# bd4/gpu-mpi-tests

Measured on AMD Instinct MI355X. Metric: 2D 5-pt Jacobi stencil MLUPS (fp64), higher is better.
Workload: dtype fp64; 1 GPU; model=mpi_stencil2d jacobi5 32768x32768 fp64, global_batch=1073741824, parallelism=spatial2d py1 x px1, serial, engine=native, hipgraph=False, temporal_blocking=True, sweeps_per_pass=20, pass_plan=98x20+1x1, exact_levels=False, init=random, transport=none, halo_bytes_per_rank=0, device=cuda:0

## Files before the change

csrc/kernels/jacobi5tb.hpp:

```cpp
#pragma once
#include <hip/hip_runtime.h>

#include <algorithm>
#include <cstdio>
#include <cstdlib>
#include <atomic>
#include <map>
#include <mutex>
#include <string>
#include <utility>
#include <vector>

#include "common.hpp"
#include "gmt/kernels.h"
#include "gmt/tb_geom.h"

namespace gmt {
namespace tb {

constexpr int kMaxRect = 8;
constexpr int kMaxThreads = 512;
constexpr uint32_t kDrop = 0x80000000u;

constexpr int unroll_for(int NL) { return NL > 1 ? 2 * (NL - 1) + 1 : 2; }
// ... 52 lines not shown
  using C = Cfg<K>;
  return static_cast<int64_t>(C::HS) * Sh<K, NW>::ROWG + static_cast<int64_t>(NW) * C::RS * C::ROW;
}

struct Args {
  int64_t r[kMaxRect][4];
  int64_t nstrip[kMaxRect];
  int64_t tstart[kMaxRect + 1];
  int64_t dom[4];
  int64_t ld;
  int64_t last_row;
  int n;
  int mask;
  int64_t e0[kMaxRect], e1[kMaxRect], nmid[kMaxRect], lmid[kMaxRect];
  int64_t nmid_b[kMaxRect], lmid_b[kMaxRect];
  int nw;
  double quarter;
  int64_t sig_wgs;
  unsigned* sig_count;
  uint64_t* signal;
  int prio;
  int rb_rect;
  int rb_s, rb_n;
  int64_t sig_rows, sig_total, sig_dispatch;
  int64_t edges_last;
  int sh;
  int shmap;
  int col_keep;
  int cb_rect;
  int cb_lo, cb_hi;
// ... 144 lines not shown
    else if constexpr (J == 2) GMT_KC("v_mov_b64 %[v2], %[c]");
    else GMT_KC("v_mov_b64 %[v3], %[c]");
  } else {
    if constexpr (J == 0) GMT_KC("v_mul_f64 %[v0], %[c], 4.0");
    else if constexpr (J == 1) GMT_KC("v_mul_f64 %[v1], %[c], 4.0");
    else if constexpr (J == 2) GMT_KC("v_mul_f64 %[v2], %[c], 4.0");
    else GMT_KC("v_mul_f64 %[v3], %[c], 4.0");
  }
#undef GMT_KC
}

#ifndef GMT_TB_SKIP_DEAD
#define GMT_TB_SKIP_DEAD 1
#endif

template <int K, int J, bool EXACT, bool EDGE, int RULE, bool UP, int PUSH, int SH>
__device__ __forceinline__ void run_stage(const Args& a, const double* __restrict__ u, double* __restrict__ un,
                                          char* ring, int lane, int64_t xs, int64_t xe, int64_t ys, int64_t ye,
                                          int nsteps, int sig_step, int xd, int64_t cf, int hdelta, uint64_t hm0,
                                          uint64_t hm1) {
  using C = Cfg<K>;
  constexpr int NC = C::NC;
  constexpr int PB = J * C::NL + 1, PE = (J + 1) * C::NL;
  constexpr bool kIn = J == 0;
  constexpr bool kOut = J == C::S - 1;
  constexpr bool SYNC = C::S > 1;
  constexpr int kP = C::P, kRS = C::RS, kHS = C::HS;
  constexpr uint32_t kRow = C::ROW;
  constexpr int D = C::DLAG * J;
  constexpr int kGroups = 1 + (PUSH & 1) + ((PUSH >> 1) & 1) + (PUSH == 3 ? 1 : 0);
  constexpr int SPS = kOut ? (EDGE ? NC : kGroups * (NC / 2)) : 0;
  static_assert(!(PUSH && EDGE), "inline halo exchange: no odd-edge stores");
  constexpr bool kDma = kIn;
  constexpr int DPS = kDma ? C::NDMA : 0;
  char* const hand_rd = ring + kRS * kRow + (J > 0 ? J - 1 : 0) * kHS * kRow;
// ... 123 lines not shown
  static_assert(RULE < 2 || kColSlot < NC, "column slot");
  const int64_t gcol = !gw && cf <= dx0 - 1 && dx0 - 1 < cf + C::COLS ? dx0 - 1 : dx1;
  const uint64_t kcm = RULE >= 2 ? __builtin_amdgcn_ballot_w64(c0 + kColSlot == gcol) : 0;

  const int64_t yanchor = up ? ye - 1 + K : yl;
  const auto clamp32 = [](int64_t x) {
    return static_cast<int>(x < INT32_MIN ? int64_t{INT32_MIN} : x > INT32_MAX ? int64_t{INT32_MAX} : x);
  };
  int tlo = up ? (gn ? INT32_MIN : clamp32(yanchor - dy1 + 1)) : (gs ? INT32_MIN : clamp32(dy0 - yanchor));
  int thi = up ? (gs ? INT32_MAX : clamp32(yanchor - dy0 + 1)) : (gn ? INT32_MAX : clamp32(dy1 - yanchor));
  if constexpr (PUSH != 0 && SH != 0) {
    tlo = __builtin_amdgcn_readfirstlane(tlo);
    thi = __builtin_amdgcn_readfirstlane(thi);
  }
  const uint32_t span = static_cast<uint32_t>(thi) - static_cast<uint32_t>(tlo);
  auto level = [&](const dv<NC>& up_, const dv<NC>& c, const dv<NC>& dn, int t) -> dv<NC> {
#pragma clang fp contract(off)
    const double w = dpp_from_lower(c.c[NC - 1]), e = dpp_from_upper(c.c[0]);
    dv<NC> v;
    static_for<0, NC>([&](auto Q) {
#pragma clang fp contract(off)
      constexpr int j = decltype(Q)::value;
      double l, r;
      if constexpr (j == 0) l = w;
      else l = c.c[j - 1];
      if constexpr (j == NC - 1) r = e;
      else r = c.c[j + 1];
      if constexpr (EXACT) v.c[j] = quarter * ((l + r) + (up_.c[j] + dn.c[j]));
      else v.c[j] = (l + r) + (up_.c[j] + dn.c[j]);
    });
    if constexpr (RULE >= 2) {
      keep_col<EXACT, kColSlot, NC>(v, c.c[kColSlot], kcm);
    } else if constexpr (RULE == 1) {
      keep_cells<EXACT, NC>(v, c, kxm, static_cast<uint32_t>(t) - static_cast<uint32_t>(tlo), span);
    }
    return v;
  };

  constexpr int NL = PE - PB + 1;
  dv<NC> W[NL > 1 ? NL - 1 : 1][2];
#pragma unroll
  for (int p = 0; p < (NL > 1 ? NL - 1 : 1); ++p)
#pragma unroll
    for (int j = 0; j < 2; ++j) W[p][j] = dv_zero<NC>();

  if constexpr (kIn) {
    static_for<0, kP>([&](auto I) {
      store_step(decltype(I)::value - kP, dv_zero<NC>());
// ... 10 lines not shown
      r2 = lds_row<NC>(ring + (s % kRS) * kRow, lane);
    } else {
      if constexpr (SH) {
        r0 = lds_row_sh<NC, kQS>(hsh + ((s + kHS - 4) % kHS) * kRowG);
        r1 = lds_row_sh<NC, kQS>(hsh + ((s + kHS - 3) % kHS) * kRowG);
        r2 = lds_row_sh<NC, kQS>(hsh + ((s + kHS - 2) % kHS) * kRowG);
      } else {
        r0 = lds_row<NC>(hand_rd + ((s + kHS - 4) % kHS) * kRow, lane);
        r1 = lds_row<NC>(hand_rd + ((s + kHS - 3) % kHS) * kRow, lane);
        r2 = lds_row<NC>(hand_rd + ((s + kHS - 2) % kHS) * kRow, lane);
      }
    }
  };
  load_rows(0);

  auto step = [&](auto Jc, int s) {
    constexpr int j = decltype(Jc)::value;
    (void)j;
    dv<NC> v = level(r0, r1, r2, s - D - PB);
    __builtin_amdgcn_sched_barrier(0);
    static_for<PB + 1, PE + 1>([&](auto Q) {
      constexpr int p = decltype(Q)::value;
      const dv<NC> nv = level(W[p - 1 - PB][0], W[p - 1 - PB][1], v, s - D - p);
      W[p - 1 - PB][0] = W[p - 1 - PB][1];
      W[p - 1 - PB][1] = v;
      v = nv;
      __builtin_amdgcn_sched_barrier(0);
    });
    if constexpr (kOut) {
      if constexpr (!EXACT) {
#pragma unroll
        for (int q = 0; q < NC; ++q) v.c[q] = __builtin_amdgcn_ldexp(v.c[q], -2 * K);
      }
      store_step(s, v);
    } else if constexpr (SH) {
      lds_put_sh<NC, kQS>(hsh + (s % kHS) * kRowG, v, hm0, hm1);
    } else {
      lds_put<NC>(hand_wr + (s % kHS) * kRow, lane, v);
// ... 2 lines not shown
    if constexpr (SYNC) asm volatile("s_waitcnt lgkmcnt(0)" ::: "memory");
    load_rows(s + 1);
    if constexpr (SYNC) asm volatile("s_barrier" ::: "memory");
  };

  constexpr int kU = C::U;
  constexpr bool kSkip0 = GMT_TB_SKIP_DEAD && !kIn && SYNC && kU <= D + 2 * PB;
  int s_first = 0;
  if constexpr (kSkip0) {
    for (int s = 0; s < kU - 1; ++s) step_barrier();
    asm volatile("s_waitcnt lgkmcnt(0)" ::: "memory");
    load_rows(kU);
    asm volatile("s_barrier" ::: "memory");
    s_first = kU;
  }
  for (int s0 = s_first; s0 < nsteps; s0 += kU) {
    static_for<0, kU>([&](auto Jc) { step(Jc, s0 + decltype(Jc)::value); });
    if constexpr (kOut) {
      if (static_cast<unsigned>(sig_step - s0) < static_cast<unsigned>(kU)) {
        asm volatile("s_waitcnt vmcnt(0)" ::: "memory");
        __builtin_amdgcn_fence(__ATOMIC_RELEASE, "agent");
        if (lane == 0 && __hip_atomic_fetch_add(a.sig_count, 1u, __ATOMIC_ACQ_REL, __HIP_MEMORY_SCOPE_AGENT) ==
                             static_cast<unsigned>(a.sig_total - 1)) {
          __hip_atomic_store(a.sig_count, 0u, __ATOMIC_RELAXED, __HIP_MEMORY_SCOPE_AGENT);
          __hip_atomic_fetch_add(a.signal, uint64_t{1}, __ATOMIC_RELEASE, __HIP_MEMORY_SCOPE_AGENT);
        }
      }
    }
  }
  wait_vmcnt<0>();
}

template <int K, bool EXACT, bool EDGE, bool PUSH, int SH>
__device__ __forceinline__ void tb_block(const Args& a, const double* __restrict__ u, double* __restrict__ un,
                                         int64_t t) {
  using C = Cfg<K>;
  constexpr int G = C::S;
  extern __shared__ d2 lds_dyn[];
  const int lane = threadIdx.x & (kWave - 1);
  const int wave = __builtin_amdgcn_readfirstlane(static_cast<int>(threadIdx.x) / kWave);
  const bool smaj = G > 1 && a.shmap;
  const int sl = smaj ? wave % a.nw : wave / G, stage = smaj ? wave / a.nw : wave % G;
  int k = 0;
  while (k + 1 < a.n && t >= a.tstart[k + 1]) ++k;
  const int64_t lt = t - a.tstart[k];
  const int64_t ngroups = (a.nstrip[k] + a.nw - 1) / a.nw;
  const int64_t ry0 = a.r[k][2], ry1 = a.r[k][2] + a.r[k][3];
  const int64_t e0 = a.e0[k], e1 = a.e1[k];
  const int64_t nedge = (e0 > 0) + (e1 > 0);
  const int rbs = k == a.rb_rect ? a.rb_s : 0, rbn = k == a.rb_rect ? a.rb_n : 0, rb = rbs + rbn;
  const int cblo = k == a.cb_rect ? a.cb_lo : 0;
  const int cbhi = k == a.cb_rect && ngroups > 1 ? a.cb_hi : 0;
  const int64_t ncb = (cblo || (k == a.cb_rect && a.cb_hi && ngroups == 1)) + cbhi;
  const int64_t nsb = nedge + a.nmid_b[k];
  const int64_t ng = ngroups - ncb;
  const int64_t cbf = ncb > 0 && (cblo || ngroups == 1) ? 1 : 0;
  const bool b0 = cbf == 0, b1 = ngroups > 1 && !cbhi;
  const int64_t nbnd = (b0 ? 1 : 0) + (b1 ? 1 : 0);
  const int64_t n_cb = ncb * nsb, n_rb = rb * ng, n_ed = nedge * ng, n_bd = (a.nmid_b[k] - rb) * nbnd;
  int64_t gi, m = -1;
  int edge = 0, dir = 1;
  bool band = false;
  auto seg_of = [&](int64_t sg, int64_t nm) {
    if (e0 > 0 && sg == 0) {
      edge = 0;
    } else if (sg < (e0 > 0) + nm) {
      m = sg - (e0 > 0);
    } else {
      edge = 1;
    }
  };
  if (lt < n_cb) {
    const int64_t c = lt / nsb;
    gi = (c == 0 && cbf) ? 0 : ngroups - 1;
    seg_of(lt % nsb, a.nmid_b[k]);
  } else if (lt < n_cb + n_rb) {
    const int64_t l0 = lt - n_cb;
    gi = cbf + l0 % ng;
    const bool north = l0 >= ng || !rbs;
    const int64_t nm = (gi == 0 || gi == ngroups - 1) ? a.nmid_b[k] : a.nmid[k];
    m = north ? nm - 1 : 0;
    dir = north ? -1 : 1;
    band = true;
  } else if (lt < n_cb + n_rb + n_ed) {
    const int64_t l1 = lt - n_cb - n_rb;
    edge = (l1 / ng == 0 && e0 > 0) ? 0 : 1;
    gi = cbf + l1 % ng;
  } else if (lt < n_cb + n_rb + n_ed + n_bd) {
    const int64_t l2 = lt - n_cb - n_rb - n_ed;
    m = rbs + l2 / nbnd;
    gi = (l2 % nbnd == 0 && b0) ? 0 : ngroups - 1;
  } else {
    const int64_t l3 = lt - n_cb - n_rb - n_ed - n_bd;
    m = rbs + l3 / (ngroups - 2);
    gi = 1 + l3 % (ngroups - 2);
  }
  const int64_t nm = (gi == 0 || gi == ngroups - 1) ? a.nmid_b[k] : a.nmid[k];
  int64_t ys, ye;
  if (m < 0) {
    ys = edge == 0 ? ry0 : ry1 - e1;
    ye = edge == 0 ? ry0 + e0 : ry1;
  } else {
    const int64_t mid = ry1 - e1 - (ry0 + e0);
    ys = ry0 + e0 + m * mid / nm;
    ye = ry0 + e0 + (m + 1) * mid / nm;
  }
  constexpr int kU = C::U;
  const int sig_step = band ? static_cast<int>(C::LAG + 2 * K + a.sig_rows - 1) : -1;
  const int nsteps = static_cast<int>((ye - ys + 2 * K + C::LAG + kU - 1) / kU * kU);
  const int64_t strip = gi * a.nw + sl;
  if (strip >= a.nstrip[k]) {
    if constexpr (G > 1) {
      for (int s = 0; s < nsteps; ++s) step_barrier();
    }
    return;
  }
  constexpr int64_t wout = C::WOUT;
  const int64_t rx0 = a.r[k][0], rx1 = a.r[k][0] + a.r[k][1];
  int64_t xs, xe, cf;
  char* ring;
// ... 18 lines not shown
    } else {
      off = H::O + H::S1 * sl;
      xs = gx + H::S1 * sl;
      xe = sl < H::NW - 1 ? xs + H::S1 : gx + H::GOUT;
    }
    cf = ga + off;
    hdelta = static_cast<int>(4 * off - (ring - lds));
  } else {
    xs = rx0 + strip * wout;
    if (xs + wout > rx1) xs = rx1 - wout > rx0 ? rx1 - wout : rx0;
    xe = xs + wout < rx1 ? xs + wout : rx1;
    cf = xs - C::KL;
    ring = reinterpret_cast<char*>(lds_dyn) + sl * strip_lds<K>();
  }
  const int64_t cx0 = cf, cx1 = cx0 + C::COLS;
  const bool rule = (cx0 < a.dom[0] && !(a.mask & 1)) || (cx1 > a.dom[0] + a.dom[1] && !(a.mask & 2)) ||
                    (ys - K < a.dom[2] && !(a.mask & 4)) || (ye + K > a.dom[2] + a.dom[3] && !(a.mask & 8));
  int rule_kind = rule ? 1 : 0;
  constexpr bool kColBodies = SH && !PUSH;
  constexpr int kJW = SH ? Sh<K, SH ? SH : 4>::kJW : 3, kJE = SH ? Sh<K, SH ? SH : 4>::kJE : 0;
  if constexpr (kColBodies) {
    const bool ry = (ys - K < a.dom[2] && !(a.mask & 4)) || (ye + K > a.dom[2] + a.dom[3] && !(a.mask & 8));
    const int64_t gw0 = a.dom[0] - 1, ge0 = a.dom[0] + a.dom[1];
    const bool hw = !(a.mask & 1) && cx0 <= gw0 && gw0 < cx1, he = !(a.mask & 2) && cx0 <= ge0 && ge0 < cx1;
    if (rule && !ry && hw != he && a.col_keep) {
      const int jslot = static_cast<int>(((hw ? gw0 : ge0) - cx0) & 3);
      if (jslot == kJW || jslot == kJE) rule_kind = 2 + jslot;
    }
  }
  const bool pw = PUSH && (a.push[GMT_PUSH_W] || a.push[GMT_PUSH_SW] || a.push[GMT_PUSH_NW]);
  const bool pe = PUSH && (a.push[GMT_PUSH_E] || a.push[GMT_PUSH_SE] || a.push[GMT_PUSH_NE]);
  const int xd = !PUSH ? -1 : (strip == 0 && pw) ? GMT_PUSH_W : (strip == a.nstrip[k] - 1 && pe) ? GMT_PUSH_E : -1;
  const bool py = PUSH && (((a.push[GMT_PUSH_S] || a.push[GMT_PUSH_SW] || a.push[GMT_PUSH_SE]) &&
                            ys < a.dom[2] + a.push_w) ||
                           ((a.push[GMT_PUSH_N] || a.push[GMT_PUSH_NW] || a.push[GMT_PUSH_NE]) &&
                            ye > a.dom[2] + a.dom[3] - a.push_w));
  const int pm = (xd >= 0 ? 1 : 0) | (py ? 2 : 0);
  using T = std::true_type;
  using F = std::false_type;
  auto go = [&](auto jc, auto rule_c, auto up_c, int sstep) __attribute__((always_inline)) {
    constexpr int j = decltype(jc)::value;
    auto run = [&](auto push_c) __attribute__((always_inline)) {
      run_stage<K, j, EXACT, EDGE, decltype(rule_c)::value, decltype(up_c)::value, decltype(push_c)::value, SH>(
          a, u, un, ring, lane, xs, xe, ys, ye, nsteps, sstep, xd, cf, hdelta, hm0, hm1);
    };
    using P0 = std::integral_constant<int, 0>;
    if constexpr (PUSH && j == G - 1) {
      if (pm != 0) run(std::integral_constant<int, 3>{});
      else run(P0{});
    } else {
      run(P0{});
    }
  };
  auto stage_go = [&](auto jc, int sstep) __attribute__((always_inline)) {
    if constexpr (!SH) {
      if (!PUSH && dir < 0) {
        if (rule) go(jc, std::integral_constant<int, 1>{}, T{}, sstep);
        else go(jc, std::integral_constant<int, 0>{}, T{}, sstep);
        return;
      }
    }
    using R0 = std::integral_constant<int, 0>;
    using R1 = std::integral_constant<int, 1>;
    if constexpr (kColBodies) {
      using RW = std::integral_constant<int, 2 + kJW>;
      using RE = std::integral_constant<int, 2 + kJE>;
      if (rule_kind == 0) go(jc, R0{}, F{}, sstep);
      else if (rule_kind == RW::value) go(jc, RW{}, F{}, sstep);
      else if (rule_kind == RE::value && RE::value != RW::value) go(jc, RE{}, F{}, sstep);
      else go(jc, R1{}, F{}, sstep);
    } else {
      if (rule) go(jc, R1{}, F{}, sstep);
      else go(jc, R0{}, F{}, sstep);
    }
  };
  if constexpr (G == 1) {
    stage_go(std::integral_constant<int, 0>{}, sig_step);
  } else {
    static_for<0, G>([&](auto Jc) __attribute__((always_inline)) {
      constexpr int j = decltype(Jc)::value;
      if (stage == j) {
        if constexpr (j == 0) {
          if (a.prio) __builtin_amdgcn_s_setprio(2);
        }
        stage_go(Jc, j == G - 1 ? sig_step : -1);
      }
    });
// ... 72 lines not shown
      __hip_atomic_fetch_add(a.signal, uint64_t{1}, __ATOMIC_RELEASE, __HIP_MEMORY_SCOPE_AGENT);
    }
  }
}

}
}
namespace {

using namespace gmt;
using namespace gmt::tb;

struct SegPlan {
  int64_t e0[kMaxRect], e1[kMaxRect], nmid[kMaxRect], lmid[kMaxRect], nmid_b[kMaxRect], lmid_b[kMaxRect];
  bool tail;
};

inline double tb_rule_cost() {
  static const double c = [] {
    const char* e = std::getenv("GMT_TB_RULE_COST");
    const double v = e ? std::atof(e) : 0.0;
    return v >= 1.0 && v <= 4.0 ? v : 1.8;
  }();
  return c;
}

inline double tb_rule_col_cost() {
  static const double c = [] {
    const char* e = std::getenv("GMT_TB_RULE_COL_COST");
    const double v = e ? std::atof(e) : 0.0;
// ... 1 lines not shown
  }();
  return c;
}

inline double tb_push_cost() {
  static const double c = [] {
    const char* e = std::getenv("GMT_TB_PUSH_COST");
    const double v = e ? std::atof(e) : 0.0;
    return v >= 1.0 && v <= 4.0 ? v : 1.3;
  }();
  return c;
}

template <int K>
SegPlan plan_segments(const Args& a, int seg_rows, int64_t lmax, int64_t resident_wgs, int sig_rects, int rb_rect = -1,
                      int rb = 0, int64_t rb_min = 0, int push_sides = 0) {
  SegPlan p{};
  const bool push_ns = (push_sides & 12) == 12;
  const double fr = tb_rule_cost(), fp = tb_push_cost();
  constexpr int64_t kWarm = 2 * K + Cfg<K>::LAG, kU = Cfg<K>::U;
  auto balanced = [](int64_t L, double f) {
    const int64_t st = (L + kWarm + kU - 1) / kU * kU;
    const int64_t blocks = static_cast<int64_t>(static_cast<double>(st) / (f * kU) + 1e-9);
    return std::max<int64_t>(64, blocks * kU - kWarm);
  };
  auto side_cost = [&](int k, double* out) {
    const int64_t ry0 = a.r[k][2], ry1 = ry0 + a.r[k][3], rx0 = a.r[k][0], rx1 = rx0 + a.r[k][1];
    const int64_t kl = a.sh ? Sh<K>::ML : Cfg<K>::KL;
    const bool rule[4] = {rx0 - kl < a.dom[0] && !(a.mask & 1), rx1 + kl > a.dom[0] + a.dom[1] && !(a.mask & 2),
                          ry0 - K < a.dom[2] && !(a.mask & 4), ry1 + K > a.dom[2] + a.dom[3] && !(a.mask & 8)};
    const double frx = a.col_keep ? tb_rule_col_cost() : fr;
    for (int d = 0; d < 4; ++d) out[d] = (rule[d] ? (d < 2 ? frx : fr) : 1.0) * ((push_sides >> d) & 1 ? fp : 1.0);
  };
  bool long_edges = false;
  auto fill = [&](int64_t L0, int64_t* wgs) {
    int64_t w = 0;
    for (int k = 0; k < a.n; ++k) {
      int64_t L = L0;
      const int64_t ny = a.r[k][3];
      if (k < sig_rects) {
        const int64_t lb = std::min<int64_t>(std::max<int64_t>(128, L - L / 4), lmax);
        p.e0[k] = p.e1[k] = 0;
        p.nmid[k] = p.nmid_b[k] = (ny + lb - 1) / lb;
        p.lmid[k] = p.lmid_b[k] = (ny + p.nmid[k] - 1) / p.nmid[k];
        w += (a.nstrip[k] + a.nw - 1) / a.nw * p.nmid[k];
        continue;
      }
      double sc[4];
      side_cost(k, sc);
      const bool top = seg_rows == 0 && sc[2] > 1.0, bot = seg_rows == 0 && sc[3] > 1.0;
      const int64_t edge0 = long_edges ? balanced(L0, sc[2]) : std::max<int64_t>(64, K);
      const int64_t edge1 = long_edges ? balanced(L0, sc[3]) : std::max<int64_t>(64, K);
      p.e0[k] = p.e1[k] = 0;
      if (ny > edge0 + edge1 + 64) {
        p.e0[k] = top ? edge0 : 0;
        p.e1[k] = bot ? edge1 : 0;
      }
      int64_t mid = ny - p.e0[k] - p.e1[k];
      if (k == rb_rect && rb > 0) L = std::min<int64_t>(L, std::max<int64_t>(rb_min, mid / rb));
      if (push_ns) L = std::min<int64_t>(L, (mid + 1) / 2);
      p.nmid[k] = (mid + L - 1) / L;
      p.lmid[k] = (mid + p.nmid[k] - 1) / p.nmid[k];
      if (long_edges && (p.e0[k] > 0 || p.e1[k] > 0)) {
        for (int it = 0; it < 4; ++it) {
          p.e0[k] = p.e0[k] > 0 ? std::min<int64_t>(balanced(p.lmid[k], sc[2]), (ny - 64) / 2) : 0;
          p.e1[k] = p.e1[k] > 0 ? std::min<int64_t>(balanced(p.lmid[k], sc[3]), (ny - 64) / 2) : 0;
          mid = ny - p.e0[k] - p.e1[k];
          p.lmid[k] = (mid + p.nmid[k] - 1) / p.nmid[k];
        }
      }
      const double fx = seg_rows == 0 ? std::max(sc[0], sc[1]) : 1.0;
      int64_t lb = fx > 1.0 ? balanced(p.lmid[k], fx) : p.lmid[k];
      if (k == rb_rect && rb > 0) lb = std::min<int64_t>(lb, std::max<int64_t>(rb_min, mid / rb));
      if (push_ns) lb = std::min<int64_t>(lb, (mid + 1) / 2);
      p.nmid_b[k] = (mid + lb - 1) / lb;
      p.lmid_b[k] = (mid + p.nmid_b[k] - 1) / p.nmid_b[k];
      const int64_t groups = (a.nstrip[k] + a.nw - 1) / a.nw, nbnd = groups < 2 ? groups : 2;
      w += groups * ((p.e0[k] > 0) + (p.e1[k] > 0)) + nbnd * p.nmid_b[k] + (groups - nbnd) * p.nmid[k];
    }
    *wgs = w;
  };
  int64_t wgs = 0;
  if (seg_rows > 0) {
    fill(std::min<int64_t>(seg_rows, lmax), &wgs);
    return p;
  }
  static const int64_t forced_l = [] {
    const char* e = std::getenv("GMT_TB_PLAN_L");
    return e ? std::max<int64_t>(0, std::atoll(e)) : int64_t(0);
  }();
  if (forced_l > 0) {
    fill(std::min<int64_t>(std::max<int64_t>(forced_l, 64), lmax), &wgs);
    return p;
// ... 6 lines not shown
    const char* e = std::getenv("GMT_TB_EDGES_LAST");
    return e ? std::atoi(e) : -1;
  }();
  const bool tail_possible = a.n == 1 && sig_rects == 0 && rb_rect < 0 && seg_rows == 0 && tail_mode != 0;
  bool tail_edges = false;
  auto makespan = [&]() {
    dur.clear();
    for (int k = 0; k < a.n; ++k) {
      const int64_t groups = (a.nstrip[k] + a.nw - 1) / a.nw, nbnd = groups < 2 ? groups : 2;
      double sc[4];
      side_cost(k, sc);
      const double fx = std::max(sc[0], sc[1]);
      const bool edges = p.e0[k] > 0 || p.e1[k] > 0;
      const double fy = edges ? 1.0 : std::max(sc[2], sc[3]);
      const double fb = std::max(fx, fy), fm = fy;
      auto edge_tiles = [&]() {
        for (int64_t g = 0; g < groups; ++g) {
          const bool bnd = g == 0 || g == groups - 1;
          if (p.e0[k] > 0) dur.push_back((bnd ? std::max(sc[2], fx) : sc[2]) * steps(p.e0[k]));
          if (p.e1[k] > 0) dur.push_back((bnd ? std::max(sc[3], fx) : sc[3]) * steps(p.e1[k]));
        }
      };
      if (!tail_edges) edge_tiles();
      for (int64_t g = 0; g < nbnd; ++g)
        for (int64_t m = 0; m < p.nmid_b[k]; ++m) dur.push_back(fb * steps(p.lmid_b[k]));
      for (int64_t g = nbnd; g < groups; ++g)
        for (int64_t m = 0; m < p.nmid[k]; ++m) dur.push_back(fm * steps(p.lmid[k]));
      if (tail_edges) edge_tiles();
    }
    const size_t ns = static_cast<size_t>(std::max<int64_t>(1, resident_wgs));
    slot.assign(std::min(ns, dur.size()), 0.0);
    size_t used = 0;
    double end = 0.0;
    auto cmp = [](double x, double y) { return x > y; };
    for (double d : dur) {
      double t0 = 0.0;
      if (used < slot.size()) {
        slot[used++] = d;
        if (used == slot.size()) std::make_heap(slot.begin(), slot.end(), cmp);
        end = std::max(end, d);
        continue;
      }
      std::pop_heap(slot.begin(), slot.end(), cmp);
      t0 = slot.back();
      slot.back() = t0 + d;
      std::push_heap(slot.begin(), slot.end(), cmp);
      end = std::max(end, t0 + d);
    }
    return end;
  };
  static const bool debug = std::getenv("GMT_TB_PLAN_DEBUG") != nullptr;
  auto eval = [&](int le, int64_t L) {
    long_edges = le == 1;
    fill(L, &wgs);
    const int64_t groups0 = (a.nstrip[0] + a.nw - 1) / a.nw;
    const int64_t ne = groups0 * ((p.e0[0] > 0) + (p.e1[0] > 0));
    const bool can_tail = tail_possible && ne > 0 && wgs - ne >= 2 * resident_wgs;
    tail_edges = false;
    double cost = makespan();
    bool tail = false;
    if (can_tail && tail_mode == 1) cost = 1e300;
    if (can_tail) {
      tail_edges = true;
      const double ct = makespan();
      if (ct < cost - 1e-9) {
        cost = ct;
        tail = true;
      }
    }
    if (debug)
      std::fprintf(stderr, "plan le %d L %lld e %lld/%lld mid %lld x %lld b %lld x %lld wgs %lld tail %d cost %.1f\n",
                   le, (long long)L, (long long)p.e0[0], (long long)p.e1[0], (long long)p.nmid[0],
                   (long long)p.lmid[0], (long long)p.nmid_b[0], (long long)p.lmid_b[0], (long long)wgs, tail ? 1 : 0,
                   cost);
    return std::make_pair(cost, tail);
  };
  const int64_t lhi = std::min<int64_t>(2048, lmax);
  int64_t best_l = 128;
  bool best_long = false, best_tail = false;
  double best = 1e300;
  static const int edges_mode = [] {
    const char* e = std::getenv("GMT_TB_EDGES");
    return e ? std::atoi(e) : 0;
  }();
  for (int le = 0; le < 2; ++le) {
    if ((edges_mode == 1 && le == 1) || (edges_mode == 2 && le == 0)) continue;
    int64_t c0 = 128;
    double b0 = 1e300;
    for (int64_t L = 128; L <= lhi; L += 16) {
      const double cost = eval(le, L).first;
      if (cost < b0 - 1e-9) {
        b0 = cost;
        c0 = L;
      }
    }
    for (int64_t L = std::max<int64_t>(128, c0 - 15); L <= std::min(lhi, c0 + 15); ++L) {
      const auto [cost, tail] = eval(le, L);
      if (cost < best - 1e-9) {
        best = cost;
        best_l = L;
        best_long = le == 1;
        best_tail = tail;
      }
    }
  }
  long_edges = best_long;
  fill(std::min<int64_t>(best_l, lmax), &wgs);
  p.tail = best_tail;
  return p;
}

template <int K, bool EXACT, bool EDGE, bool PUSH, int SH>
int launch_tb(const gmt_tb_opts& o, int n_rect, const int64_t* rects, const int64_t* dom, int mask, const double* u,
              double* un, int64_t ld, int64_t nrows, hipStream_t s, int64_t* info = nullptr) {
  using C = Cfg<K>;
  constexpr int G = C::S;
  constexpr int kMaxStrips = tb_max_strips(K);
  Args a{};
  a.nw = std::min(o.wg_waves > 0 ? o.wg_waves : tb_default_strips(K), kMaxStrips);
  static const int col_keep = [] {
    const char* e = std::getenv("GMT_TB_COL_KEEP");
    return e ? std::atoi(e) : 1;
  }();
// ... 91 lines not shown
  if (o.reserved_cus > 0) {
    int cus = 256;
    (void)hipDeviceGetAttribute(&cus, hipDeviceAttributeMultiprocessorCount, dev);
    if (o.reserved_cus < cus) per_cu = static_cast<int>(static_cast<int64_t>(per_cu) * (cus - o.reserved_cus) / cus);
  }
  const int sig_rects = o.signal_rects;
  const int cbk = (o.signal_cols & 3) ? sig_rects : -1;
  if (cbk >= a.n) return static_cast<int>(hipErrorInvalidValue);
  const int rbk = o.signal_rows > 0 ? sig_rects : -1;
  const int rbs = rbk >= 0 && (mask & 4) ? 1 : 0, rbn = rbk >= 0 && (mask & 8) ? 1 : 0;
  const int64_t rb_min = std::max<int64_t>(32, o.signal_rows);
  if (rbk >= 0 && (rbk >= a.n || rbs + rbn == 0 || a.r[rbk][3] < (rbs + rbn) * rb_min))
    return static_cast<int>(hipErrorInvalidValue);
  SegPlan sp;
  {
    std::vector<int64_t> key = {a.n, a.nw, a.mask, o.seg_rows, lmax, per_cu, sig_rects, rbk, rbs + rbn, rb_min, push_sides, SH};
    for (int k = 0; k < a.n; ++k) key.insert(key.end(), a.r[k], a.r[k] + 4);
    key.insert(key.end(), a.dom, a.dom + 4);
    static std::mutex mu;
    static std::map<std::vector<int64_t>, SegPlan> cache;
    std::lock_guard<std::mutex> g(mu);
    auto it = cache.find(key);
    if (it == cache.end()) {
      if (cache.size() > 256) cache.clear();
      it = cache.emplace(key, plan_segments<K>(a, o.seg_rows, lmax, per_cu, sig_rects, rbk, rbs + rbn, rb_min, push_sides)).first;
    }
    sp = it->second;
  }
  a.tstart[0] = 0;
  for (int k = 0; k < a.n; ++k) {
    a.e0[k] = sp.e0[k];
    a.e1[k] = sp.e1[k];
    a.nmid[k] = sp.nmid[k];
    a.lmid[k] = sp.lmid[k];
    a.nmid_b[k] = sp.nmid_b[k];
    a.lmid_b[k] = sp.lmid_b[k];
    const int64_t groups = (a.nstrip[k] + a.nw - 1) / a.nw, nbnd = groups < 2 ? groups : 2;
    a.tstart[k + 1] = a.tstart[k] + groups * ((sp.e0[k] > 0) + (sp.e1[k] > 0)) + nbnd * sp.nmid_b[k] +
                      (groups - nbnd) * sp.nmid[k];
  }
  for (int k = a.n + 1; k <= kMaxRect; ++k) a.tstart[k] = a.tstart[a.n];
  const int64_t nb = a.tstart[a.n];
  a.sig_wgs = a.tstart[sig_rects];
  a.rb_rect = -1;
  a.cb_rect = -1;
  int64_t cb_groups = 0, cb_strips = 0;
  if (cbk >= 0) {
    const int64_t groups = (a.nstrip[cbk] + a.nw - 1) / a.nw;
    a.cb_rect = cbk;
    a.cb_lo = (o.signal_cols & 1) ? 1 : 0;
    a.cb_hi = (o.signal_cols & 2) ? 1 : 0;
    cb_groups = groups == 1 ? 1 : a.cb_lo + a.cb_hi;
    if (groups == 1) cb_strips = a.nstrip[cbk];
    else cb_strips = (a.cb_lo ? std::min<int64_t>(a.nw, a.nstrip[cbk]) : 0) +
// ... 10 lines not shown
      return static_cast<int>(hipErrorInvalidValue);
    a.rb_rect = rbk;
    a.rb_s = rbs;
    a.rb_n = rbn;
    a.sig_rows = o.signal_rows;
    const int64_t groups = (a.nstrip[rbk] + a.nw - 1) / a.nw;
    const bool cbr = rbk == cbk;
    a.sig_total += rb * (a.nstrip[rbk] - (cbr ? cb_strips : 0));
    a.sig_dispatch += rb * (groups - (cbr ? cb_groups : 0));
  }
  static const bool special_rr = [] {
    const char* e = std::getenv("GMT_TB_SPECIAL_RR");
    return e && std::atoi(e) > 0;
  }();
  if (sp.tail && a.n == 1 && a.sig_dispatch == 0) {
    const int64_t groups = (a.nstrip[0] + a.nw - 1) / a.nw;
    const int64_t ne = groups * ((sp.e0[0] > 0) + (sp.e1[0] > 0));
    if (tail_swizzle_ok(nb, ne)) a.edges_last = ne;
  }
  if (special_rr && a.n == 1 && a.sig_dispatch == 0) {
    const int64_t groups = (a.nstrip[0] + a.nw - 1) / a.nw, nbnd = groups < 2 ? groups : 2;
    a.sig_dispatch = groups * ((sp.e0[0] > 0) + (sp.e1[0] > 0)) + nbnd * sp.nmid_b[0];
  }
  static const int prio_mode = [] {
    const char* e = std::getenv("GMT_TB_PRIO");
    return e ? std::atoi(e) : -1;
  }();
  a.prio = prio_mode >= 0 ? (prio_mode > 0 ? 1 : 0) : (nb <= per_cu ? 1 : 0);
  a.sig_count = o.signal_count;
  a.signal = o.signal;
  a.stop = PUSH ? o.stop : nullptr;
  a.clk = o.clock;
  if (info) {
    hipFuncAttributes fa{};
    (void)hipFuncGetAttributes(&fa, reinterpret_cast<const void*>(&jacobi5tb_kernel<K, EXACT, EDGE, PUSH, SH>));
    const int64_t v[6] = {nb, per_cu, a.nw * G * kWave, a.lmid[0], a.nmid[0], fa.numRegs};
    for (int j = 0; j < 6; ++j) info[j] = v[j];
// ... 143 lines not shown
```

Before: 5.227 million MLUPS.

## Apply boundary rule only over prefix steps and plan tiles without boundary edges

```diff
diff --git a/csrc/kernels/jacobi5tb.hpp b/csrc/kernels/jacobi5tb.hpp
--- a/csrc/kernels/jacobi5tb.hpp
+++ b/csrc/kernels/jacobi5tb.hpp
@@ -90,6 +90,7 @@
   int mask;
   int64_t e0[kMaxRect], e1[kMaxRect], nmid[kMaxRect], lmid[kMaxRect];
   int64_t nmid_b[kMaxRect], lmid_b[kMaxRect];
+  int noedge_b;
   int nw;
   double quarter;
   int64_t sig_wgs;
@@ -264,11 +265,20 @@
 #define GMT_TB_SKIP_DEAD 1
 #endif
 
+#ifndef GMT_TB_RULE_PREFIX
+#define GMT_TB_RULE_PREFIX 1
+#endif
+constexpr bool tb_rule_prefix_built(int K, bool sh) {
+  return GMT_TB_RULE_PREFIX != 0 && K != 10 && !(K == 20 && sh);
+}
+
+constexpr int kRuleSplit = -1;
+
 template <int K, int J, bool EXACT, bool EDGE, int RULE, bool UP, int PUSH, int SH>
 __device__ __forceinline__ void run_stage(const Args& a, const double* __restrict__ u, double* __restrict__ un,
                                           char* ring, int lane, int64_t xs, int64_t xe, int64_t ys, int64_t ye,
                                           int nsteps, int sig_step, int xd, int64_t cf, int hdelta, uint64_t hm0,
-                                          uint64_t hm1) {
+                                          uint64_t hm1, int rmode = 0) {
   using C = Cfg<K>;
   constexpr int NC = C::NC;
   constexpr int PB = J * C::NL + 1, PE = (J + 1) * C::NL;
@@ -422,8 +432,9 @@
     thi = __builtin_amdgcn_readfirstlane(thi);
   }
   const uint32_t span = static_cast<uint32_t>(thi) - static_cast<uint32_t>(tlo);
-  auto level = [&](const dv<NC>& up_, const dv<NC>& c, const dv<NC>& dn, int t) -> dv<NC> {
+  auto level = [&](auto Rc, const dv<NC>& up_, const dv<NC>& c, const dv<NC>& dn, int t) -> dv<NC> {
 #pragma clang fp contract(off)
+    constexpr int kRule = decltype(Rc)::value;
     const double w = dpp_from_lower(c.c[NC - 1]), e = dpp_from_upper(c.c[0]);
     dv<NC> v;
     static_for<0, NC>([&](auto Q) {
@@ -437,9 +448,9 @@
       if constexpr (EXACT) v.c[j] = quarter * ((l + r) + (up_.c[j] + dn.c[j]));
       else v.c[j] = (l + r) + (up_.c[j] + dn.c[j]);
     });
-    if constexpr (RULE >= 2) {
+    if constexpr (kRule >= 2) {
       keep_col<EXACT, kColSlot, NC>(v, c.c[kColSlot], kcm);
-    } else if constexpr (RULE == 1) {
+    } else if constexpr (kRule == 1) {
       keep_cells<EXACT, NC>(v, c, kxm, static_cast<uint32_t>(t) - static_cast<uint32_t>(tlo), span);
     }
     return v;
@@ -480,14 +491,12 @@
   };
   load_rows(0);
 
-  auto step = [&](auto Jc, int s) {
-    constexpr int j = decltype(Jc)::value;
-    (void)j;
-    dv<NC> v = level(r0, r1, r2, s - D - PB);
+  auto step = [&](auto Rc, int s) {
+    dv<NC> v = level(Rc, r0, r1, r2, s - D - PB);
     __builtin_amdgcn_sched_barrier(0);
     static_for<PB + 1, PE + 1>([&](auto Q) {
       constexpr int p = decltype(Q)::value;
-      const dv<NC> nv = level(W[p - 1 - PB][0], W[p - 1 - PB][1], v, s - D - p);
+      const dv<NC> nv = level(Rc, W[p - 1 - PB][0], W[p - 1 - PB][1], v, s - D - p);
       W[p - 1 - PB][0] = W[p - 1 - PB][1];
       W[p - 1 - PB][1] = v;
       v = nv;
@@ -520,8 +529,18 @@
     asm volatile("s_barrier" ::: "memory");
     s_first = kU;
   }
-  for (int s0 = s_first; s0 < nsteps; s0 += kU) {
-    static_for<0, kU>([&](auto Jc) { step(Jc, s0 + decltype(Jc)::value); });
+  int rule_end = 0;
+  if constexpr (RULE == kRuleSplit) {
+    if (rmode == 1) {
+      rule_end = nsteps;
+    } else if (rmode == 2) {
+      const int64_t e = static_cast<int64_t>(tlo) + D + PE;
+      rule_end = e <= 0 ? 0 : e >= nsteps ? nsteps : static_cast<int>((e + kU - 1) / kU * kU);
+    }
+    rule_end = __builtin_amdgcn_readfirstlane(rule_end);
+  }
+  auto block = [&](auto Rc, int s0) __attribute__((always_inline)) {
+    static_for<0, kU>([&](auto I) { step(Rc, s0 + decltype(I)::value); });
     if constexpr (kOut) {
       if (static_cast<unsigned>(sig_step - s0) < static_cast<unsigned>(kU)) {
         asm volatile("s_waitcnt vmcnt(0)" ::: "memory");
@@ -533,7 +552,12 @@
         }
       }
     }
-  }
+  };
+  int s0 = s_first;
+  if constexpr (RULE == kRuleSplit) {
+    for (; s0 < rule_end; s0 += kU) block(std::integral_constant<int, 1>{}, s0);
+  }
+  for (; s0 < nsteps; s0 += kU) block(std::integral_constant<int, RULE == kRuleSplit ? 0 : RULE>{}, s0);
   wait_vmcnt<0>();
 }
 
@@ -563,7 +587,9 @@
   const int64_t cbf = ncb > 0 && (cblo || ngroups == 1) ? 1 : 0;
   const bool b0 = cbf == 0, b1 = ngroups > 1 && !cbhi;
   const int64_t nbnd = (b0 ? 1 : 0) + (b1 ? 1 : 0);
-  const int64_t n_cb = ncb * nsb, n_rb = rb * ng, n_ed = nedge * ng, n_bd = (a.nmid_b[k] - rb) * nbnd;
+  const bool noeb = a.noedge_b != 0;
+  const int64_t nge = noeb ? ngroups - nbnd : ng, ge0 = noeb ? 1 : cbf;
+  const int64_t n_cb = ncb * nsb, n_rb = rb * ng, n_ed = nedge * nge, n_bd = (a.nmid_b[k] - rb) * nbnd;
   int64_t gi, m = -1;
   int edge = 0, dir = 1;
   bool band = false;
@@ -590,8 +616,8 @@
     band = true;
   } else if (lt < n_cb + n_rb + n_ed) {
     const int64_t l1 = lt - n_cb - n_rb;
-    edge = (l1 / ng == 0 && e0 > 0) ? 0 : 1;
-    gi = cbf + l1 % ng;
+    edge = (l1 / nge == 0 && e0 > 0) ? 0 : 1;
+    gi = ge0 + l1 % nge;
   } else if (lt < n_cb + n_rb + n_ed + n_bd) {
     const int64_t l2 = lt - n_cb - n_rb - n_ed;
     m = rbs + l2 / nbnd;
@@ -607,9 +633,11 @@
     ys = edge == 0 ? ry0 : ry1 - e1;
     ye = edge == 0 ? ry0 + e0 : ry1;
   } else {
-    const int64_t mid = ry1 - e1 - (ry0 + e0);
-    ys = ry0 + e0 + m * mid / nm;
-    ye = ry0 + e0 + (m + 1) * mid / nm;
+    const bool whole = noeb && (gi == 0 || gi == ngroups - 1);
+    const int64_t f0 = whole ? 0 : e0, f1 = whole ? 0 : e1;
+    const int64_t mid = ry1 - f1 - (ry0 + f0);
+    ys = ry0 + f0 + m * mid / nm;
+    ye = ry0 + f0 + (m + 1) * mid / nm;
   }
   constexpr int kU = C::U;
   const int sig_step = band ? static_cast<int>(C::LAG + 2 * K + a.sig_rows - 1) : -1;
@@ -658,8 +686,14 @@
     ring = reinterpret_cast<char*>(lds_dyn) + sl * strip_lds<K>();
   }
   const int64_t cx0 = cf, cx1 = cx0 + C::COLS;
-  const bool rule = (cx0 < a.dom[0] && !(a.mask & 1)) || (cx1 > a.dom[0] + a.dom[1] && !(a.mask & 2)) ||
-                    (ys - K < a.dom[2] && !(a.mask & 4)) || (ye + K > a.dom[2] + a.dom[3] && !(a.mask & 8));
+  const bool rule_x = (cx0 < a.dom[0] && !(a.mask & 1)) || (cx1 > a.dom[0] + a.dom[1] && !(a.mask & 2));
+  const bool rule_s = ys - K < a.dom[2] && !(a.mask & 4), rule_n = ye + K > a.dom[2] + a.dom[3] && !(a.mask & 8);
+  const bool rule = rule_x || rule_s || rule_n;
+  constexpr bool kRulePrefix = tb_rule_prefix_built(K, SH != 0);
+  if constexpr (kRulePrefix && !SH && !PUSH) {
+    if (rule_n && !rule_s && !rule_x && !band) dir = -1;
+  }
+  const int rmode = !rule ? 0 : (rule_x || (dir < 0 ? rule_s || !rule_n : rule_n || !rule_s)) ? 1 : 2;
   int rule_kind = rule ? 1 : 0;
   constexpr bool kColBodies = SH && !PUSH;
   constexpr int kJW = SH ? Sh<K, SH ? SH : 4>::kJW : 3, kJE = SH ? Sh<K, SH ? SH : 4>::kJE : 0;
@@ -684,37 +718,53 @@
   using F = std::false_type;
   auto go = [&](auto jc, auto rule_c, auto up_c, int sstep) __attribute__((always_inline)) {
     constexpr int j = decltype(jc)::value;
-    auto run = [&](auto push_c) __attribute__((always_inline)) {
-      run_stage<K, j, EXACT, EDGE, decltype(rule_c)::value, decltype(up_c)::value, decltype(push_c)::value, SH>(
-          a, u, un, ring, lane, xs, xe, ys, ye, nsteps, sstep, xd, cf, hdelta, hm0, hm1);
+    auto run = [&](auto rc, auto push_c) __attribute__((always_inline)) {
+      run_stage<K, j, EXACT, EDGE, decltype(rc)::value, decltype(up_c)::value, decltype(push_c)::value, SH>(
+          a, u, un, ring, lane, xs, xe, ys, ye, nsteps, sstep, xd, cf, hdelta, hm0, hm1, rmode);
     };
     using P0 = std::integral_constant<int, 0>;
     if constexpr (PUSH && j == G - 1) {
-      if (pm != 0) run(std::integral_constant<int, 3>{});
-      else run(P0{});
+      using P3 = std::integral_constant<int, 3>;
+      if (pm != 0) {
+        if constexpr (decltype(rule_c)::value == kRuleSplit) {
+          if (rule) run(std::integral_constant<int, 1>{}, P3{});
+          else run(std::integral_constant<int, 0>{}, P3{});
+        } else {
+          run(rule_c, P3{});
+        }
+      } else {
+        run(rule_c, P0{});
+      }
     } else {
-      run(P0{});
+      run(rule_c, P0{});
     }
   };
   auto stage_go = [&](auto jc, int sstep) __attribute__((always_inline)) {
     if constexpr (!SH) {
       if (!PUSH && dir < 0) {
-        if (rule) go(jc, std::integral_constant<int, 1>{}, T{}, sstep);
-        else go(jc, std::integral_constant<int, 0>{}, T{}, sstep);
+        if constexpr (kRulePrefix) {
+          go(jc, std::integral_constant<int, kRuleSplit>{}, T{}, sstep);
+        } else {
+          if (rule) go(jc, std::integral_constant<int, 1>{}, T{}, sstep);
+          else go(jc, std::integral_constant<int, 0>{}, T{}, sstep);
+        }
         return;
       }
     }
     using R0 = std::integral_constant<int, 0>;
     using R1 = std::integral_constant<int, 1>;
+    using RS = std::integral_constant<int, kRuleSplit>;
     if constexpr (kColBodies) {
       using RW = std::integral_constant<int, 2 + kJW>;
       using RE = std::integral_constant<int, 2 + kJE>;
-      if (rule_kind == 0) go(jc, R0{}, F{}, sstep);
-      else if (rule_kind == RW::value) go(jc, RW{}, F{}, sstep);
+      if (rule_kind == RW::value) go(jc, RW{}, F{}, sstep);
       else if (rule_kind == RE::value && RE::value != RW::value) go(jc, RE{}, F{}, sstep);
+      else if constexpr (kRulePrefix) go(jc, RS{}, F{}, sstep);
+      else if (rule_kind == 0) go(jc, R0{}, F{}, sstep);
       else go(jc, R1{}, F{}, sstep);
     } else {
-      if (rule) go(jc, R1{}, F{}, sstep);
+      if constexpr (kRulePrefix) go(jc, RS{}, F{}, sstep);
+      else if (rule) go(jc, R1{}, F{}, sstep);
       else go(jc, R0{}, F{}, sstep);
     }
   };
@@ -817,6 +867,7 @@
 struct SegPlan {
   int64_t e0[kMaxRect], e1[kMaxRect], nmid[kMaxRect], lmid[kMaxRect], nmid_b[kMaxRect], lmid_b[kMaxRect];
   bool tail;
+  bool noedge_b;
 };
 
 inline double tb_rule_cost() {
@@ -848,7 +899,7 @@
 
 template <int K>
 SegPlan plan_segments(const Args& a, int seg_rows, int64_t lmax, int64_t resident_wgs, int sig_rects, int rb_rect = -1,
-                      int rb = 0, int64_t rb_min = 0, int push_sides = 0) {
+                      int rb = 0, int64_t rb_min = 0, int push_sides = 0, bool col_bands = false) {
   SegPlan p{};
   const bool push_ns = (push_sides & 12) == 12;
   const double fr = tb_rule_cost(), fp = tb_push_cost();
@@ -858,6 +909,17 @@
     const int64_t blocks = static_cast<int64_t>(static_cast<double>(st) / (f * kU) + 1e-9);
     return std::max<int64_t>(64, blocks * kU - kWarm);
   };
+  constexpr int64_t kRuleSteps = (kWarm + kU - 1) / kU * kU;
+  const bool kRulePrefix = tb_rule_prefix_built(K, a.sh != 0);
+  const bool prefix[2] = {kRulePrefix && push_sides == 0, false};
+  auto prefix_cost = [&](double st) { return st + (fr - 1.0) * std::min<double>(st, kRuleSteps); };
+  auto balanced_prefix = [&](int64_t L) {
+    const int64_t st = (L + kWarm + kU - 1) / kU * kU;
+    const double room = static_cast<double>(st) - (fr - 1.0) * kRuleSteps;
+    const int64_t blocks = room >= kRuleSteps ? static_cast<int64_t>(room / kU + 1e-9)
+                                              : static_cast<int64_t>(static_cast<double>(st) / (fr * kU) + 1e-9);
+    return std::max<int64_t>(64, blocks * kU - kWarm);
+  };
   auto side_cost = [&](int k, double* out) {
     const int64_t ry0 = a.r[k][2], ry1 = ry0 + a.r[k][3], rx0 = a.r[k][0], rx1 = rx0 + a.r[k][1];
     const int64_t kl = a.sh ? Sh<K>::ML : Cfg<K>::KL;
@@ -866,8 +928,16 @@
     const double frx = a.col_keep ? tb_rule_col_cost() : fr;
     for (int d = 0; d < 4; ++d) out[d] = (rule[d] ? (d < 2 ? frx : fr) : 1.0) * ((push_sides >> d) & 1 ? fp : 1.0);
   };
-  bool long_edges = false;
+  int edge_mode = 0;
+  const bool can_noeb = kRulePrefix && push_sides == 0 && a.n == 1 && sig_rects == 0 && rb_rect < 0 && !col_bands &&
+                        seg_rows == 0;
+  bool noeb = false;
+  auto edge_len = [&](int64_t L, const double* sc, int side) {
+    const bool px = prefix[side] && sc[2 + side] > 1.0 && (noeb || std::max(sc[0], sc[1]) <= 1.0);
+    return px ? balanced_prefix(L) : balanced(L, sc[2 + side]);
+  };
   auto fill = [&](int64_t L0, int64_t* wgs) {
+    const bool long_edges = edge_mode == 1;
     int64_t w = 0;
     for (int k = 0; k < a.n; ++k) {
       int64_t L = L0;
@@ -882,9 +952,10 @@
       }
       double sc[4];
       side_cost(k, sc);
-      const bool top = seg_rows == 0 && sc[2] > 1.0, bot = seg_rows == 0 && sc[3] > 1.0;
-      const int64_t edge0 = long_edges ? balanced(L0, sc[2]) : std::max<int64_t>(64, K);
-      const int64_t edge1 = long_edges ? balanced(L0, sc[3]) : std::max<int64_t>(64, K);
+      const bool top = seg_rows == 0 && edge_mode != 2 && sc[2] > 1.0;
+      const bool bot = seg_rows == 0 && edge_mode != 2 && sc[3] > 1.0;
+      const int64_t edge0 = long_edges ? edge_len(L0, sc, 0) : std::max<int64_t>(64, K);
+      const int64_t edge1 = long_edges ? edge_len(L0, sc, 1) : std::max<int64_t>(64, K);
       p.e0[k] = p.e1[k] = 0;
       if (ny > edge0 + edge1 + 64) {
         p.e0[k] = top ? edge0 : 0;
@@ -897,8 +968,8 @@
       p.lmid[k] = (mid + p.nmid[k] - 1) / p.nmid[k];
       if (long_edges && (p.e0[k] > 0 || p.e1[k] > 0)) {
         for (int it = 0; it < 4; ++it) {
-          p.e0[k] = p.e0[k] > 0 ? std::min<int64_t>(balanced(p.lmid[k], sc[2]), (ny - 64) / 2) : 0;
-          p.e1[k] = p.e1[k] > 0 ? std::min<int64_t>(balanced(p.lmid[k], sc[3]), (ny - 64) / 2) : 0;
+          p.e0[k] = p.e0[k] > 0 ? std::min<int64_t>(edge_len(p.lmid[k], sc, 0), (ny - 64) / 2) : 0;
+          p.e1[k] = p.e1[k] > 0 ? std::min<int64_t>(edge_len(p.lmid[k], sc, 1), (ny - 64) / 2) : 0;
           mid = ny - p.e0[k] - p.e1[k];
           p.lmid[k] = (mid + p.nmid[k] - 1) / p.nmid[k];
         }
@@ -907,10 +978,12 @@
       int64_t lb = fx > 1.0 ? balanced(p.lmid[k], fx) : p.lmid[k];
       if (k == rb_rect && rb > 0) lb = std::min<int64_t>(lb, std::max<int64_t>(rb_min, mid / rb));
       if (push_ns) lb = std::min<int64_t>(lb, (mid + 1) / 2);
-      p.nmid_b[k] = (mid + lb - 1) / lb;
-      p.lmid_b[k] = (mid + p.nmid_b[k] - 1) / p.nmid_b[k];
+      const int64_t mid_b = noeb ? ny : mid;
+      p.nmid_b[k] = (mid_b + lb - 1) / lb;
+      p.lmid_b[k] = (mid_b + p.nmid_b[k] - 1) / p.nmid_b[k];
       const int64_t groups = (a.nstrip[k] + a.nw - 1) / a.nw, nbnd = groups < 2 ? groups : 2;
-      w += groups * ((p.e0[k] > 0) + (p.e1[k] > 0)) + nbnd * p.nmid_b[k] + (groups - nbnd) * p.nmid[k];
+      w += (noeb ? groups - nbnd : groups) * ((p.e0[k] > 0) + (p.e1[k] > 0)) + nbnd * p.nmid_b[k] +
+           (groups - nbnd) * p.nmid[k];
     }
     *wgs = w;
   };
@@ -947,18 +1020,40 @@
       const bool edges = p.e0[k] > 0 || p.e1[k] > 0;
       const double fy = edges ? 1.0 : std::max(sc[2], sc[3]);
       const double fb = std::max(fx, fy), fm = fy;
+      auto row_tile = [&](int side, bool bnd, double st) {
+        if (prefix[side] && sc[2 + side] > 1.0 && !(bnd && fx > 1.0)) return prefix_cost(st);
+        return std::max(sc[2 + side], bnd ? fx : 1.0) * st;
+      };
       auto edge_tiles = [&]() {
         for (int64_t g = 0; g < groups; ++g) {
           const bool bnd = g == 0 || g == groups - 1;
-          if (p.e0[k] > 0) dur.push_back((bnd ? std::max(sc[2], fx) : sc[2]) * steps(p.e0[k]));
-          if (p.e1[k] > 0) dur.push_back((bnd ? std::max(sc[3], fx) : sc[3]) * steps(p.e1[k]));
+          if (bnd && noeb) continue;
+          if (p.e0[k] > 0) dur.push_back(row_tile(0, bnd, steps(p.e0[k])));
+          if (p.e1[k] > 0) dur.push_back(row_tile(1, bnd, steps(p.e1[k])));
         }
       };
       if (!tail_edges) edge_tiles();
-      for (int64_t g = 0; g < nbnd; ++g)
-        for (int64_t m = 0; m < p.nmid_b[k]; ++m) dur.push_back(fb * steps(p.lmid_b[k]));
-      for (int64_t g = nbnd; g < groups; ++g)
-        for (int64_t m = 0; m < p.nmid[k]; ++m) dur.push_back(fm * steps(p.lmid[k]));
+      if (kRulePrefix && push_sides == 0) {
+        auto mid_tiles = [&](int64_t ng, int64_t nm, int64_t lm, bool bnd) {
+          const bool s0 = (p.e0[k] == 0 || (bnd && noeb)) && sc[2] > 1.0, s1 = (p.e1[k] == 0 || (bnd && noeb)) && sc[3] > 1.0;
+          const double st = steps(lm), f0 = bnd ? fx : 1.0;
+          for (int64_t m = 0; m < nm; ++m) {
+            const bool t0 = s0 && m == 0, t1 = s1 && m == nm - 1;
+            const double d = t0 && t1 ? std::max({f0, sc[2], sc[3]}) * st
+                             : t0     ? row_tile(0, bnd, st)
+                             : t1     ? row_tile(1, bnd, st)
+                                      : f0 * st;
+            for (int64_t g = 0; g < ng; ++g) dur.push_back(d);
+          }
+        };
+        mid_tiles(nbnd, p.nmid_b[k], p.lmid_b[k], true);
+        mid_tiles(groups - nbnd, p.nmid[k], p.lmid[k], false);
+      } else {
+        for (int64_t g = 0; g < nbnd; ++g)
+          for (int64_t m = 0; m < p.nmid_b[k]; ++m) dur.push_back(fb * steps(p.lmid_b[k]));
+        for (int64_t g = nbnd; g < groups; ++g)
+          for (int64_t m = 0; m < p.nmid[k]; ++m) dur.push_back(fm * steps(p.lmid[k]));
+      }
       if (tail_edges) edge_tiles();
     }
     const size_t ns = static_cast<size_t>(std::max<int64_t>(1, resident_wgs));
@@ -984,10 +1079,10 @@
   };
   static const bool debug = std::getenv("GMT_TB_PLAN_DEBUG") != nullptr;
   auto eval = [&](int le, int64_t L) {
-    long_edges = le == 1;
+    edge_mode = le;
     fill(L, &wgs);
     const int64_t groups0 = (a.nstrip[0] + a.nw - 1) / a.nw;
-    const int64_t ne = groups0 * ((p.e0[0] > 0) + (p.e1[0] > 0));
+    const int64_t ne = (noeb ? groups0 - std::min<int64_t>(groups0, 2) : groups0) * ((p.e0[0] > 0) + (p.e1[0] > 0));
     const bool can_tail = tail_possible && ne > 0 && wgs - ne >= 2 * resident_wgs;
     tail_edges = false;
     double cost = makespan();
@@ -1002,22 +1097,31 @@
       }
     }
     if (debug)
-      std::fprintf(stderr, "plan le %d L %lld e %lld/%lld mid %lld x %lld b %lld x %lld wgs %lld tail %d cost %.1f\n",
-                   le, (long long)L, (long long)p.e0[0], (long long)p.e1[0], (long long)p.nmid[0],
+      std::fprintf(stderr, "plan le %d noeb %d L %lld e %lld/%lld mid %lld x %lld b %lld x %lld wgs %lld tail %d cost %.1f\n",
+                   le, noeb ? 1 : 0, (long long)L, (long long)p.e0[0], (long long)p.e1[0], (long long)p.nmid[0],
                    (long long)p.lmid[0], (long long)p.nmid_b[0], (long long)p.lmid_b[0], (long long)wgs, tail ? 1 : 0,
                    cost);
     return std::make_pair(cost, tail);
   };
   const int64_t lhi = std::min<int64_t>(2048, lmax);
   int64_t best_l = 128;
-  bool best_long = false, best_tail = false;
+  int best_mode = 0;
+  bool best_tail = false;
   double best = 1e300;
   static const int edges_mode = [] {
     const char* e = std::getenv("GMT_TB_EDGES");
     return e ? std::atoi(e) : 0;
   }();
-  for (int le = 0; le < 2; ++le) {
-    if ((edges_mode == 1 && le == 1) || (edges_mode == 2 && le == 0)) continue;
+  const bool try_none = (prefix[0] || prefix[1]) && sig_rects == 0 && rb_rect < 0;
+  double sc0[4];
+  side_cost(0, sc0);
+  const bool try_noeb = can_noeb && std::max(sc0[0], sc0[1]) > 1.0 && std::max(sc0[2], sc0[3]) > 1.0;
+  bool best_noeb = false;
+  for (int lm = 0; lm < (try_noeb ? 5 : 3); ++lm) {
+    const int le = lm < 3 ? lm : lm - 3;
+    if (le == 2 && !try_none) continue;
+    if (edges_mode > 0 && le != edges_mode - 1) continue;
+    noeb = lm >= 3;
     int64_t c0 = 128;
     double b0 = 1e300;
     for (int64_t L = 128; L <= lhi; L += 16) {
@@ -1032,14 +1136,17 @@
       if (cost < best - 1e-9) {
         best = cost;
         best_l = L;
-        best_long = le == 1;
+        best_mode = le;
         best_tail = tail;
-      }
-    }
-  }
-  long_edges = best_long;
+        best_noeb = noeb;
+      }
+    }
+  }
+  edge_mode = best_mode;
+  noeb = best_noeb;
   fill(std::min<int64_t>(best_l, lmax), &wgs);
   p.tail = best_tail;
+  p.noedge_b = best_noeb && (p.e0[0] > 0 || p.e1[0] > 0);
   return p;
 }
 
@@ -1161,7 +1268,7 @@
     return static_cast<int>(hipErrorInvalidValue);
   SegPlan sp;
   {
-    std::vector<int64_t> key = {a.n, a.nw, a.mask, o.seg_rows, lmax, per_cu, sig_rects, rbk, rbs + rbn, rb_min, push_sides, SH};
+    std::vector<int64_t> key = {a.n, a.nw, a.mask, o.seg_rows, lmax, per_cu, sig_rects, rbk, rbs + rbn, rb_min, push_sides, SH, cbk};
     for (int k = 0; k < a.n; ++k) key.insert(key.end(), a.r[k], a.r[k] + 4);
     key.insert(key.end(), a.dom, a.dom + 4);
     static std::mutex mu;
@@ -1170,10 +1277,12 @@
     auto it = cache.find(key);
     if (it == cache.end()) {
       if (cache.size() > 256) cache.clear();
-      it = cache.emplace(key, plan_segments<K>(a, o.seg_rows, lmax, per_cu, sig_rects, rbk, rbs + rbn, rb_min, push_sides)).first;
+      it = cache.emplace(key, plan_segments<K>(a, o.seg_rows, lmax, per_cu, sig_rects, rbk, rbs + rbn, rb_min, push_sides,
+                                               cbk >= 0)).first;
     }
     sp = it->second;
   }
+  a.noedge_b = sp.noedge_b && a.n == 1 && sig_rects == 0 && rbk < 0 && cbk < 0 ? 1 : 0;
   a.tstart[0] = 0;
   for (int k = 0; k < a.n; ++k) {
     a.e0[k] = sp.e0[k];
@@ -1183,8 +1292,8 @@
     a.nmid_b[k] = sp.nmid_b[k];
     a.lmid_b[k] = sp.lmid_b[k];
     const int64_t groups = (a.nstrip[k] + a.nw - 1) / a.nw, nbnd = groups < 2 ? groups : 2;
-    a.tstart[k + 1] = a.tstart[k] + groups * ((sp.e0[k] > 0) + (sp.e1[k] > 0)) + nbnd * sp.nmid_b[k] +
-                      (groups - nbnd) * sp.nmid[k];
+    a.tstart[k + 1] = a.tstart[k] + (a.noedge_b ? groups - nbnd : groups) * ((sp.e0[k] > 0) + (sp.e1[k] > 0)) +
+                      nbnd * sp.nmid_b[k] + (groups - nbnd) * sp.nmid[k];
   }
   for (int k = a.n + 1; k <= kMaxRect; ++k) a.tstart[k] = a.tstart[a.n];
   const int64_t nb = a.tstart[a.n];
@@ -1225,13 +1334,13 @@
     return e && std::atoi(e) > 0;
   }();
   if (sp.tail && a.n == 1 && a.sig_dispatch == 0) {
-    const int64_t groups = (a.nstrip[0] + a.nw - 1) / a.nw;
-    const int64_t ne = groups * ((sp.e0[0] > 0) + (sp.e1[0] > 0));
+    const int64_t groups = (a.nstrip[0] + a.nw - 1) / a.nw, nbnd = groups < 2 ? groups : 2;
+    const int64_t ne = (a.noedge_b ? groups - nbnd : groups) * ((sp.e0[0] > 0) + (sp.e1[0] > 0));
     if (tail_swizzle_ok(nb, ne)) a.edges_last = ne;
   }
   if (special_rr && a.n == 1 && a.sig_dispatch == 0) {
     const int64_t groups = (a.nstrip[0] + a.nw - 1) / a.nw, nbnd = groups < 2 ? groups : 2;
-    a.sig_dispatch = groups * ((sp.e0[0] > 0) + (sp.e1[0] > 0)) + nbnd * sp.nmid_b[0];
+    a.sig_dispatch = (a.noedge_b ? groups - nbnd : groups) * ((sp.e0[0] > 0) + (sp.e1[0] > 0)) + nbnd * sp.nmid_b[0];
   }
   static const int prio_mode = [] {
     const char* e = std::getenv("GMT_TB_PRIO");
```

Measured after the change: 5.241 million MLUPS (median of 3 runs). About the same (+0.3%).
